# nanoshimarobot/dynamic_direct_lidar_odometry

Measured on AMD Instinct MI355X. Metric: GICP iters/sec + ms/scan, 131k-pt source → 500k-pt submap; pose Δ vs CPU ref, higher is better.
Workload: dtype f32 search / f64 normal equations; 1 GPU; cfg3 S2M GICP: 131,072-pt 64x2048 scan -> 500,000-pt 4-keyframe submap, LM, maxCorr 2.0 m, maxIter 32, transEps 0.01; target_points=500000, parallelism=replicas x1

## Files before the change

### dynamic_direct_lidar_odometry_amd/csrc/moments.hip

```cpp
#include <hip/hip_runtime.h>

#include <cstddef>

#include "gicp_types.hpp"
#include "search.hpp"
#include "nftree.hpp"
#include "cov_math.hpp"
#include "launch.hpp"
#include "launch_util.hpp"
#include "linearize_internal.hpp"
#include "lm_step.hpp"

namespace ddlo {

struct Contrib {
  double M[6];
  double q[3];
  double qq[6];
  double v[3];
  double y;
  double c;
};

template <int S>
__device__ __forceinline__ double moment_val(const Contrib& C) {
  if constexpr (S < 6) {
    return C.M[S];
  } else if constexpr (S < 24) {
    return C.q[(S - 6) / 6] * C.M[(S - 6) % 6];
  } else if constexpr (S < 60) {
    return C.qq[(S - 24) / 6] * C.M[(S - 24) % 6];
  } else if constexpr (S < 72) {
    constexpr int m = (S - 60) / 4, kk = (S - 60) % 4;
    if constexpr (kk == 3)
      return C.v[m];
    else
      return C.v[m] * C.q[kk];
  } else if constexpr (S == 72) {
    return C.y;
  } else if constexpr (S == 73) {
    return C.c;
  } else {
    return 0.0;
  }
}

__device__ __forceinline__ double dpp_f64(double x, int ctrl_sel) {
  const int lo = __double2loint(x), hi = __double2hiint(x);
  int rlo, rhi;
  switch (ctrl_sel) {
    case 0:
      rlo = __builtin_amdgcn_update_dpp(0, lo, 0x140, 0xf, 0xf, false);
      rhi = __builtin_amdgcn_update_dpp(0, hi, 0x140, 0xf, 0xf, false);
      break;
    case 1:
      rlo = __builtin_amdgcn_update_dpp(0, lo, 0x141, 0xf, 0xf, false);
      rhi = __builtin_amdgcn_update_dpp(0, hi, 0x141, 0xf, 0xf, false);
      break;
    case 2:
      rlo = __builtin_amdgcn_update_dpp(0, lo, 0x4e, 0xf, 0xf, false);
      rhi = __builtin_amdgcn_update_dpp(0, hi, 0x4e, 0xf, 0xf, false);
      break;
    default:
      rlo = __builtin_amdgcn_update_dpp(0, lo, 0xb1, 0xf, 0xf, false);
      rhi = __builtin_amdgcn_update_dpp(0, hi, 0xb1, 0xf, 0xf, false);
      break;
  }
  return __hiloint2double(rhi, rlo);
}

template <int L>
__device__ __forceinline__ double xchg(double a, double b) {
  if constexpr (L == 1 || L == 2) {
    const unsigned alo = __double2loint(a), ahi = __double2hiint(a);
    const unsigned blo = __double2loint(b), bhi = __double2hiint(b);
    unsigned x0, x1, y0, y1;
    if constexpr (L == 1) {
      const auto rl = __builtin_amdgcn_permlane32_swap(alo, blo, false, false);
      const auto rh = __builtin_amdgcn_permlane32_swap(ahi, bhi, false, false);
      x0 = rl[0]; y0 = rl[1]; x1 = rh[0]; y1 = rh[1];
    } else {
      const auto rl = __builtin_amdgcn_permlane16_swap(alo, blo, false, false);
      const auto rh = __builtin_amdgcn_permlane16_swap(ahi, bhi, false, false);
      x0 = rl[0]; y0 = rl[1]; x1 = rh[0]; y1 = rh[1];
    }
    return __hiloint2double(x1, x0) + __hiloint2double(y1, y0);
  } else {
    const int bit = 1 << (6 - L);
    const bool hi = (lane_id() & bit) != 0;
    const double keep = hi ? b : a;
    const double send = hi ? a : b;
    return keep + dpp_f64(send, L - 3);
  }
}

template <int L, int S>
__device__ __forceinline__ double treduce(const Contrib& C) {
  if constexpr (L == 0) {
    return moment_val<S>(C);
  } else {
    constexpr int half = kMomentSlots >> L;
    const double a = treduce<L - 1, S>(C);
    const double b = treduce<L - 1, S + half>(C);
    return xchg<L>(a, b);
  }
}

__device__ __forceinline__ double final_pair(double x) { return x + dpp_f64(x, 3); }

__device__ __forceinline__ int moment_base(int lane) {
  return 48 * ((lane >> 5) & 1) + 24 * ((lane >> 4) & 1) + 12 * ((lane >> 3) & 1) + 6 * ((lane >> 2) & 1) +
         3 * ((lane >> 1) & 1);
}

__device__ __forceinline__ void load_sym6(const __attribute__((address_space(1))) double* p, double c[6]) {
  const auto q = (const __attribute__((address_space(1))) d2v*)p;
  const d2v a = q[0];
  const d2v b = q[1];
  const d2v d = q[2];
  c[0] = a.x; c[1] = a.y; c[2] = b.x; c[3] = b.y; c[4] = d.x; c[5] = d.y;
}

constexpr int kMomWaves = 8;

__device__ __forceinline__ void resolve_tied_corr(const AlignJob* __restrict__ job, AlignState* st, const CloudDev& tgt,
                                               bool tied, int i, float kd, int& j, NfWaveStack* S,
                                               bool q_in_regs = false, float qx = 0.f, float qy = 0.f, float qz = 0.f) {
  unsigned long long tm = __ballot(tied);
  const int lane = lane_id();
  const NfTreeDev t = job->tgt_nf;
  if (t.nodes == nullptr) {
    if (lane == __builtin_ctzll(tm)) atomicOr(&st->tie_pending, 1);
    return;
  }
  if (*job->tgt_nf_status) {
    if (lane == __builtin_ctzll(tm)) atomicOr(&st->tie_err, 2);
    return;
  }
  int nres = 0;
  while (tm) {
    const int l = __builtin_ctzll(tm);
    tm &= tm - 1;
    const int il = __builtin_amdgcn_readlane(i, l);
    const float dl = __uint_as_float((unsigned)__builtin_amdgcn_readlane((int)__float_as_uint(kd), l));
    const float4 q = q_in_regs ? make_float4(readlane_f(qx, l), readlane_f(qy, l), readlane_f(qz, l), 0.f)
                               : ldg4(job->qstate, il);
    float rd;
    int rix;
    int err = 0, jn = -1;
    const bool ok = nf_search_wave(t, q.x, q.y, q.z, 1, S, &rd, &rix);
    rd = __uint_as_float((unsigned)__builtin_amdgcn_readfirstlane((int)__float_as_uint(rd)));
    rix = __builtin_amdgcn_readfirstlane(rix);
    if (!ok) err = 1;
    else if (__float_as_uint(rd) != __float_as_uint(dl) || rix < 0 || rix >= t.n) err = 16;
    else if ((jn = tgt.inv_perm[rix]) < 0) err = 32;
    if (lane == l) {
      if (jn >= 0) j = jn;
      else atomicOr(&st->tie_err, err);
    }
    ++nres;
  }
  if (lane == 0) atomicAdd(&st->ties_resolved, nres);
}

#ifndef DDLO_LOOKUP_U
#define DDLO_LOOKUP_U 16
#endif
constexpr int kLookupU = DDLO_LOOKUP_U;

#ifdef DDLO_MOM_PROF
#define MOM_PROF(i) if (LOOKUP) mp_t[i] = __builtin_amdgcn_s_memrealtime()
constexpr int kMomProfIters = 8, kMomProfWaves = 2048;
__device__ unsigned long long g_mom_prof[kMomProfIters * kMomProfWaves * 6];
#else
#define MOM_PROF(i)
#endif
struct TieWords {
  int pending, resolved, err;
};
constexpr int kTieThread = 64 * (kMomWaves - 1);
__device__ __forceinline__ TieWords fetch_tie_words(AlignState* st) {
  TieWords tw{0, 0, 0};
  __hip_atomic_compare_exchange_strong(&st->tie_pending, &tw.pending, 0, __ATOMIC_RELAXED, __ATOMIC_RELAXED,
                                       __HIP_MEMORY_SCOPE_AGENT);
  __hip_atomic_compare_exchange_strong(&st->ties_resolved, &tw.resolved, 0, __ATOMIC_RELAXED, __ATOMIC_RELAXED,
                                       __HIP_MEMORY_SCOPE_AGENT);
  __hip_atomic_compare_exchange_strong(&st->tie_err, &tw.err, 0, __ATOMIC_RELAXED, __ATOMIC_RELAXED,
                                       __HIP_MEMORY_SCOPE_AGENT);
  return tw;
}

__device__ __forceinline__ void publish_state(const AlignJob* __restrict__ job, AlignState* __restrict__ st,
                                              AlignState* __restrict__ publish, const TieWords& tw) {
  static_assert(sizeof(AlignState) % 8 == 0, "AlignState is copied in 8-byte words");
  static_assert(offsetof(AlignState, pub) == sizeof(AlignState) - 8, "the publication word is the last 8 bytes");
  static_assert(offsetof(AlignState, iter) % 8 == 0 && offsetof(AlignState, done) == offsetof(AlignState, iter) + 4,
                "iter and done are one 8-byte word");
  __shared__ int tie_s[3];
  if (threadIdx.x == kTieThread) {
    tie_s[0] = tw.pending;
    tie_s[1] = tw.resolved;
    tie_s[2] = tw.err;
  }
  asm volatile("s_waitcnt vmcnt(0)" ::: "memory");
  __syncthreads();
  const auto src = gpw(reinterpret_cast<unsigned long long*>(st));
  const auto dst = gpw(reinterpret_cast<unsigned long long*>(publish));
  constexpr int kWords = (int)(sizeof(AlignState) / 8);
  static_assert(kWords <= 64 * kMomWaves && kLmThreads == 64 * kMomWaves, "one 8-byte word per thread");
  auto patch = [](unsigned long long v, int w, size_t off, int val) {
    if ((size_t)w != off / 8) return v;
    const int sh = (int)(off & 4) * 8;
    return (v & ~(0xffffffffull << sh)) | ((unsigned long long)(unsigned)val << sh);
  };
  __shared__ unsigned long long iter_s;
  const int w = threadIdx.x;
  if (w < kWords) {
    unsigned long long v = __hip_atomic_load(src + w, __ATOMIC_RELAXED, __HIP_MEMORY_SCOPE_AGENT);
    v = patch(v, w, offsetof(AlignState, tie_pending), tie_s[0]);
    v = patch(v, w, offsetof(AlignState, ties_resolved), tie_s[1]);
    v = patch(v, w, offsetof(AlignState, tie_err), tie_s[2]);
    dst[w] = v;
    if (w == (int)(offsetof(AlignState, iter) / 8)) iter_s = v;
  }
  const unsigned long long tk = job->ticket;
  asm volatile("s_waitcnt vmcnt(0)" ::: "memory");
  __syncthreads();
  if (threadIdx.x == 0) {
    const unsigned long long id = iter_s;
    const unsigned long long w = (tk << 17) | ((unsigned long long)((unsigned)(id >> 32) != 0u) << 16) | (id & 0xffffu);
    __hip_atomic_store(&publish->pub, w, __ATOMIC_RELEASE, __HIP_MEMORY_SCOPE_SYSTEM);
  }
}

template <bool FUSE_LM, bool LOOKUP = false>
__global__ __launch_bounds__(64 * kMomWaves) void k_moments(const AlignJob* __restrict__ job,
                                                            AlignState* __restrict__ st, AlignState* __restrict__ publish) {
#ifdef DDLO_MOM_PROF
  unsigned long long mp_t[6] = {0, 0, 0, 0, 0, 0};
#endif
  MOM_PROF(0);
  const auto sg = gp(st);
  double R[9], t[3];
  for (int e = 0; e < 9; ++e) R[e] = sg->R[e];
  for (int e = 0; e < 3; ++e) t[e] = sg->t[e];
  const int st_rec = sg->rec, st_any_rec = sg->any_rec;
  if (__builtin_amdgcn_readfirstlane(sg->done)) {
    if (FUSE_LM && publish && blockIdx.x == 0) {
      TieWords tw{};
      if (threadIdx.x == kTieThread) tw = fetch_tie_words(st);
      publish_state(job, st, publish, tw);
    }
    return;
  }
  const CloudDev src = job->src;
  const CloudDev tgt = job->tgt;
  const auto src_cov = gp(job->src_cov);
  const auto tgt_cov = gp(job->tgt_cov);
  const auto key = gp((const unsigned long long*)job->key);
  const auto corr = gpw(job->corr);
  const auto sqd = gpw(job->sqd);
  const auto slab = gpw(job->slab);
  const double max_corr2 = job->max_corr2;
  const int rec = st_rec;
  const int first_rec_done = st_any_rec;
  const int tie_detect = job->tie_detect;
  const bool slice_check = tie_detect && job->tie_scan >= 2 && !(job->tie_ab & 4);
  const bool tie3m = tie_detect && job->tie_scan == 3 && !rec;
  __shared__ NfWaveStack tie_stk[kMomWaves];
  const int lane = lane_id();
  const int wib = threadIdx.x >> 6;
#ifdef DDLO_MOM_PROF
  __builtin_amdgcn_s_waitcnt(0);
#endif
  MOM_PROF(1);
  const int wave = blockIdx.x * kMomWaves + wib;
  const int nwaves_total = gridDim.x * kMomWaves;
  const int ngroups = (src.n + 63) >> 6;
  if (blockIdx.x == 0 && threadIdx.x < kTaskRegions) job->task_ctr[threadIdx.x * kCtrStride] = 0u;
  if (blockIdx.x == 0 && job->grid_on && threadIdx.x == 0) {
    unsigned t = 0;
    for (int sg = 0; sg < kFbSegs; ++sg) t += job->fb_count[sg * 32];
    job->fb_count[kFbSegs * 32] += t;
    for (int sg = 0; sg < kFbSegs; ++sg) job->fb_count[sg * 32] = 0u;
  }
  double acc0 = 0.0, acc1 = 0.0, acc2 = 0.0;
  for (int g = wave; g < ngroups; g += nwaves_total) {
    const int i = g * 64 + lane;
    const bool active = i < src.n;
    int j = -1;
    unsigned kj = 0xffffffffu;
    float kd = INFINITY;
    bool tied = false;
    float4 a = make_float4(0.f, 0.f, 0.f, 0.f), b = a;
    double ca[6] = {0, 0, 0, 0, 0, 0}, cb[6] = {0, 0, 0, 0, 0, 0};
    float lqx = 0.f, lqy = 0.f, lqz = 0.f;
    unsigned long long lkey = 0ull;
    unsigned lsec = 0xffffffffu;
    if constexpr (LOOKUP) {
      const CellGridDev G = job->grid;
      a = ldg4(src.pts, active ? i : src.n - 1);
      const float Rf0 = (float)R[0], Rf1 = (float)R[1], Rf2 = (float)R[2], Rf3 = (float)R[3], Rf4 = (float)R[4],
                  Rf5 = (float)R[5], Rf6 = (float)R[6], Rf7 = (float)R[7], Rf8 = (float)R[8];
      const float tf0 = (float)t[0], tf1 = (float)t[1], tf2 = (float)t[2];
      lqx = (Rf0 * a.x + Rf1 * a.y) + (Rf2 * a.z + tf0);
      lqy = (Rf3 * a.x + Rf4 * a.y) + (Rf5 * a.z + tf1);
      lqz = (Rf6 * a.x + Rf7 * a.y) + (Rf8 * a.z + tf2);
      const int g16 = i >> 4;
      const float qa = job->own_axis == 0 ? lqx : job->own_axis == 1 ? lqy : lqz;
      const bool owned = active && (job->own_axis < 0 || (qa >= job->own_lo && qa < job->own_hi)) &&
                         (job->own_mod == 0 || (g16 % job->own_mod) == job->own_rem);
      unsigned off = 0, cnt = 0;
      if (owned) {
        const float tx = (lqx - G.ox) * G.inv_s, ty = (lqy - G.oy) * G.inv_s, tz = (lqz - G.oz) * G.inv_s;
        if (tx >= 0.f && tx < (float)G.nx && ty >= 0.f && ty < (float)G.ny && tz >= 0.f && tz < (float)G.nz) {
          cg_cell_list(G, tx, ty, tz, off, cnt);
        }
      }
      unsigned long long bk = ~0ull;
      float d2 = INFINITY, bx = 0.f, by = 0.f, bz = 0.f;
      const bool track2 = tie_detect;
      constexpr int kU = kLookupU;
      auto consume = [&](const float4 (&pp)[kU], unsigned k) {
#pragma unroll
        for (int u = 0; u < kU; ++u) {
          if (k + u < cnt) {
            const float dd = dist2(lqx, lqy, lqz, pp[u].x, pp[u].y, pp[u].z);
            const unsigned long long kk = dkey(dd, __float_as_int(pp[u].w));
            if (kk < bk) {
              if (track2 && bk != ~0ull) d2 = fminf(d2, __uint_as_float((unsigned)(bk >> 32)));
              bk = kk;
              bx = pp[u].x;
              by = pp[u].y;
              bz = pp[u].z;
            } else if (track2) {
              d2 = fminf(d2, dd);
            }
          }
        }
      };
      auto fetch = [&](float4 (&pp)[kU], unsigned k) {
#pragma unroll
        for (int u = 0; u < kU; ++u) pp[u] = ldg4(G.ent, off + min(k + u, cnt - 1));
      };
      for (unsigned k = 0; k < cnt; k += kU) {
        float4 pp[kU];
        fetch(pp, k);
        consume(pp, k);
      }
      lkey = owned ? umin64(bk, dkey(job->cap2, -1)) : dkey(INFINITY, -1);
      const float lkd = __uint_as_float((unsigned)(lkey >> 32));
      lsec = (owned && (unsigned)lkey != 0xffffffffu && d2 == lkd) ? (unsigned)(lkey >> 32) : 0xffffffffu;
      b = make_float4(bx, by, bz, 0.f);

      MOM_PROF(2);
    }
    if (active) {
      const unsigned long long k = LOOKUP ? lkey : key[i];
      const unsigned sv = !tie_detect ? 0xffffffffu : LOOKUP ? lsec : job->sec[i];
      const unsigned k2lo = (tie3m && !LOOKUP) ? (unsigned)job->key2[i] : 0u;
      kj = (unsigned)k;
      kd = __uint_as_float((unsigned)(k >> 32));
      j = (kj != 0xffffffffu && (double)kd < max_corr2) ? (int)kj : -1;
      if (j >= 0) {
        if constexpr (!LOOKUP) {
          a = ldg4(src.pts, i);
          b = ldg4(tgt.pts, j);
        }

        load_sym6(src_cov + 6 * (size_t)i, ca);
        load_sym6(tgt_cov + 6 * (size_t)j, cb);
      }
      const bool searched = tie_detect && j >= 0 && sv != 0xffffffffu;
      tied = searched && sv <= (unsigned)(k >> 32);
      if (tie3m && searched && !LOOKUP) tied = tied || k2lo != ((unsigned)k ^ 0xffffffffu);
      if (slice_check && searched && !tied) {
        const float qx = ((float)R[0] * a.x + (float)R[1] * a.y) + ((float)R[2] * a.z + (float)t[0]);
        const float qy = ((float)R[3] * a.x + (float)R[4] * a.y) + ((float)R[5] * a.z + (float)t[1]);
        const float qz = ((float)R[6] * a.x + (float)R[7] * a.y) + ((float)R[8] * a.z + (float)t[2]);
        const int b0 = j & ~7;
#pragma unroll
        for (int h = 0; h < 8; ++h) {
          const float4 p = ldg4(tgt.pts, b0 + h);
          tied = tied || (b0 + h != j && dist2(qx, qy, qz, p.x, p.y, p.z) == kd);
        }
      }
    }
    if (tie_detect && __any(tied)) {
      const int j0 = j;
      resolve_tied_corr(job, st, tgt, tied, i, kd, j, &tie_stk[wib], LOOKUP, lqx, lqy, lqz);
      if (tied) kj = (unsigned)j;
      if (j != j0) {
        b = ldg4(tgt.pts, j);
        load_sym6(tgt_cov + 6 * (size_t)j, cb);
      }
    }
    if (active) {
      corr[i] = j;
      sqd[i] = kj != 0xffffffffu ? kd : INFINITY;
      if (rec && !LOOKUP) {
        const float4 qs = ldg4(job->qstate, i);
        if (qs.w >= 0.f) {
          job->ref[i] = make_float4(qs.x, qs.y, qs.z, fminf(__uint_as_float(job->sec[i]), qs.w));
          float4 pp = make_float4(0.f, 0.f, 0.f, __int_as_float(-1));
          if (kj != 0xffffffffu) {
            const float4 p = ldg4(tgt.pts, (int)kj);
            pp = make_float4(p.x, p.y, p.z, __int_as_float((int)kj));
          }
          job->ref_p[i] = pp;
        } else if (!first_rec_done) {
          job->ref[i] = make_float4(0.f, 0.f, 0.f, -1.f);
        }
      }
    }
    Contrib C;
    if (j >= 0) {
      const double A[9] = {ca[0], ca[1], ca[2], ca[1], ca[3], ca[4], ca[2], ca[4], ca[5]};
      double RC[9];
#pragma unroll
      for (int r = 0; r < 3; ++r)
#pragma unroll
        for (int cc = 0; cc < 3; ++cc) RC[3 * r + cc] = R[3 * r] * A[cc] + R[3 * r + 1] * A[3 + cc] + R[3 * r + 2] * A[6 + cc];
      double S[9];
#pragma unroll
      for (int r = 0; r < 3; ++r)
#pragma unroll
        for (int cc = 0; cc < 3; ++cc) S[3 * r + cc] = RC[3 * r] * R[3 * cc] + RC[3 * r + 1] * R[3 * cc + 1] + RC[3 * r + 2] * R[3 * cc + 2];
      const double Cm[9] = {cb[0] + S[0], cb[1] + S[1], cb[2] + S[2], cb[1] + S[3], cb[3] + S[4],
                            cb[4] + S[5], cb[2] + S[6], cb[4] + S[7], cb[5] + S[8]};
      double Mi[9];
      inv3(Cm, Mi);
      C.M[0] = Mi[0]; C.M[1] = 0.5 * (Mi[1] + Mi[3]); C.M[2] = 0.5 * (Mi[2] + Mi[6]);
      C.M[3] = Mi[4]; C.M[4] = 0.5 * (Mi[5] + Mi[7]); C.M[5] = Mi[8];
      const double ax = a.x, ay = a.y, az = a.z;
      C.q[0] = (R[0] * ax + R[1] * ay) + (R[2] * az + t[0]);
      C.q[1] = (R[3] * ax + R[4] * ay) + (R[5] * az + t[1]);
      C.q[2] = (R[6] * ax + R[7] * ay) + (R[8] * az + t[2]);
      const double e0 = (double)b.x - C.q[0], e1 = (double)b.y - C.q[1], e2 = (double)b.z - C.q[2];
      C.v[0] = C.M[0] * e0 + C.M[1] * e1 + C.M[2] * e2;
      C.v[1] = C.M[1] * e0 + C.M[3] * e1 + C.M[4] * e2;
      C.v[2] = C.M[2] * e0 + C.M[4] * e1 + C.M[5] * e2;
      C.y = e0 * C.v[0] + e1 * C.v[1] + e2 * C.v[2];
      C.c = 1.0;
    } else {
      for (int e = 0; e < 6; ++e) C.M[e] = 0.0;
      C.q[0] = C.q[1] = C.q[2] = 0.0;
      C.v[0] = C.v[1] = C.v[2] = 0.0;
      C.y = 0.0;
      C.c = 0.0;
    }
    C.qq[0] = C.q[0] * C.q[0]; C.qq[1] = C.q[0] * C.q[1]; C.qq[2] = C.q[0] * C.q[2];
    C.qq[3] = C.q[1] * C.q[1]; C.qq[4] = C.q[1] * C.q[2]; C.qq[5] = C.q[2] * C.q[2];
    MOM_PROF(3);
    acc0 += final_pair(treduce<5, 0>(C));
    acc1 += final_pair(treduce<5, 1>(C));
    acc2 += final_pair(treduce<5, 2>(C));
  }
  MOM_PROF(4);
  __shared__ double red[kMomWaves][kMomentSlots];
  if ((lane & 1) == 0) {
    const int base = moment_base(lane);
    red[wib][base + 0] = acc0;
    red[wib][base + 1] = acc1;
    red[wib][base + 2] = acc2;
  }
  __syncthreads();
  if (threadIdx.x < kSlabStride) {
    double sum = 0.0;
    if (threadIdx.x < kMoments)
      for (int w = 0; w < kMomWaves; ++w) sum += red[w][threadIdx.x];
    if constexpr (FUSE_LM)
      __hip_atomic_store((__attribute__((address_space(1))) unsigned long long*)(slab + (size_t)blockIdx.x * kSlabStride +
                                                                                 threadIdx.x),
                         (unsigned long long)__double_as_longlong(sum), __ATOMIC_RELAXED, __HIP_MEMORY_SCOPE_AGENT);
    else
      slab[(size_t)blockIdx.x * kSlabStride + threadIdx.x] = sum;
  }
#ifdef DDLO_MOM_PROF
  MOM_PROF(5);
  if (LOOKUP && lane == 0 && wave < kMomProfWaves) {
    unsigned long long* o = g_mom_prof + ((size_t)min(st->iter, kMomProfIters - 1) * kMomProfWaves + wave) * 6;
    for (int e = 0; e < 6; ++e) o[e] = mp_t[e];
  }
#endif
  if constexpr (FUSE_LM) {
    __shared__ int last_s;
    asm volatile("s_waitcnt vmcnt(0)" ::: "memory");
    __syncthreads();
    unsigned* const arrive = job->task_ctr + kTaskRegions * kCtrStride;
    if (threadIdx.x == 0) last_s = atomicAdd(arrive, 1u) == gridDim.x - 1;
    __syncthreads();
    if (!last_s) return;
    if (threadIdx.x == 0) {
      __builtin_amdgcn_fence(__ATOMIC_ACQUIRE, "agent");
      asm volatile("s_waitcnt vmcnt(0)" ::: "memory");
      atomicExch(arrive, 0u);
    }
    __syncthreads();
    TieWords tw{};
    if (publish && threadIdx.x == kTieThread) tw = fetch_tie_words(st);
    lm_step_body<false>(job, st, job->slab, job->nblocks, nullptr);
    if (publish) publish_state(job, st, publish, tw);
  }
}
template __global__ void k_moments<false>(const AlignJob*, AlignState*, AlignState*);
template __global__ void k_moments<true>(const AlignJob*, AlignState*, AlignState*);
template __global__ void k_moments<false, true>(const AlignJob*, AlignState*, AlignState*);
template __global__ void k_moments<true, true>(const AlignJob*, AlignState*, AlignState*);

__global__ __launch_bounds__(kLmThreads) void k_mom_reduce(const AlignJob* __restrict__ job) {
  AlignState* st = job->state;
  if (__builtin_amdgcn_readfirstlane(st->done)) return;
  __shared__ double part[kLmParts][kSlabStride];
  __shared__ double mom[kSlabStride];
  reduce_slab(job->slab, job->nblocks, part, mom);
  __syncthreads();
  if (threadIdx.x < kSlabStride) gpw(job->mom)[threadIdx.x] = mom[threadIdx.x];
}

__global__ __launch_bounds__(kLmThreads) void k_lm_step(const AlignJob* __restrict__ job, AlignState* __restrict__ st,
                                                        const double* __restrict__ slab, int nblocks,
                                                        const double* __restrict__ premom,
                                                        AlignState* __restrict__ publish) {
  TieWords tw{};
  if (publish && threadIdx.x == kTieThread) tw = fetch_tie_words(st);
  if (!__builtin_amdgcn_readfirstlane(st->done)) {
    if (premom) lm_step_body<true>(job, st, slab, nblocks, premom);
    else lm_step_body<false>(job, st, slab, nblocks, nullptr);
  }
  if (publish) publish_state(job, st, publish, tw);
}

void launch_linearize(hipStream_t s, const AlignJob* job, const LinGeom& g, AlignState* publish) {
  static const int fused_lookup = env_knob("DDLO_GRID_FUSED", 1);
  if (g.grid && !g.grid_walk && fused_lookup) {
    if (g.fuse_lm) k_moments<true, true><<<g.mom_blocks, 64 * kMomWaves, 0, s>>>(job, g.state, publish);
    else k_moments<false, true><<<g.mom_blocks, 64 * kMomWaves, 0, s>>>(job, g.state, nullptr);
    return;
  }
  if (g.grid) launch_cell_lookup(s, job, g);
  if (!g.grid || g.grid_walk) launch_nn_walk(s, job, g);
  if (g.fuse_lm) k_moments<true><<<g.mom_blocks, 64 * kMomWaves, 0, s>>>(job, g.state, publish);
  else k_moments<false><<<g.mom_blocks, 64 * kMomWaves, 0, s>>>(job, g.state, nullptr);
}
int moment_blocks(int nsrc) {
  const int groups = (nsrc + 63) / 64;
  return std::max(1, std::min((groups + kMomWaves - 1) / kMomWaves, kMomBlocksMax));
}
int lm_slab_rows_max() { return kMomBlocksMax; }
void launch_lm_step(hipStream_t s, const AlignJob* job, AlignState* st, const double* slab, int nblocks,
                    const double* premom, AlignState* publish) {
  k_lm_step<<<1, kLmThreads, 0, s>>>(job, st, slab, nblocks, premom, publish);
}
void launch_mom_reduce(hipStream_t s, const AlignJob* job) { k_mom_reduce<<<1, kLmThreads, 0, s>>>(job); }

}

#ifdef DDLO_MOM_PROF
extern "C" int ddlo_dev_mom_prof(unsigned long long* out) {
  return (int)hipMemcpyFromSymbol(out, HIP_SYMBOL(ddlo::g_mom_prof), sizeof(ddlo::g_mom_prof));
}
#endif
```

Measured before the change: 31860 GICP iters/s.

## Split heavy-cell candidate scans across lane teams with shuffle merge

Each lane first scans up to the first 32 candidates of its grid cell list. Lanes whose cells hold more candidates are collected per wave by ballot, and each is assigned a power-of-two team of lanes that scan the remaining candidates in strided chunks. Partial bests are merged back through shuffles, keeping the tie-tracking second distance. This aims to cut wave divergence, where a few lanes with long cell lists stall the whole wave, at the cost of extra shuffles and team bookkeeping in the lookup path.

```diff
diff --git a/dynamic_direct_lidar_odometry_amd/csrc/moments.hip b/dynamic_direct_lidar_odometry_amd/csrc/moments.hip
--- a/dynamic_direct_lidar_odometry_amd/csrc/moments.hip
+++ b/dynamic_direct_lidar_odometry_amd/csrc/moments.hip
@@ -167,11 +167,51 @@
 #define DDLO_LOOKUP_U 16
 #endif
 constexpr int kLookupU = DDLO_LOOKUP_U;
+#ifndef DDLO_TAIL_E0
+#define DDLO_TAIL_E0 32
+#endif
+#ifndef DDLO_TAIL_FCAP
+#define DDLO_TAIL_FCAP 64
+#endif
+constexpr unsigned kTailE0 = DDLO_TAIL_E0;
+constexpr int kTailFCap = DDLO_TAIL_FCAP;
+static_assert(kTailE0 > 0 && kTailE0 % kLookupU == 0, "the common rounds end on a round boundary");
+static_assert(kTailFCap >= 1 && kTailFCap <= 64 && (kTailFCap & (kTailFCap - 1)) == 0, "team size: a power of two");
+
+struct LookupBest {
+  unsigned long long bk;
+  float d2, bx, by, bz;
+};
+__device__ __forceinline__ void tail_merge(LookupBest& a, const LookupBest& o, bool track2) {
+  const bool take = o.bk < a.bk;
+  const unsigned long long loser = take ? a.bk : o.bk;
+  if (take) {
+    a.bk = o.bk;
+    a.bx = o.bx;
+    a.by = o.by;
+    a.bz = o.bz;
+  }
+  if (track2) {
+    a.d2 = fminf(a.d2, o.d2);
+    if (loser != ~0ull) a.d2 = fminf(a.d2, __uint_as_float((unsigned)(loser >> 32)));
+  }
+}
+__device__ __forceinline__ LookupBest tail_shfl(const LookupBest& s, int src) {
+  LookupBest r;
+  r.bk = ((unsigned long long)(unsigned)__shfl((int)(unsigned)(s.bk >> 32), src) << 32) |
+         (unsigned)__shfl((int)(unsigned)s.bk, src);
+  r.d2 = __shfl(s.d2, src);
+  r.bx = __shfl(s.bx, src);
+  r.by = __shfl(s.by, src);
+  r.bz = __shfl(s.bz, src);
+  return r;
+}
 
 #ifdef DDLO_MOM_PROF
 #define MOM_PROF(i) if (LOOKUP) mp_t[i] = __builtin_amdgcn_s_memrealtime()
 constexpr int kMomProfIters = 8, kMomProfWaves = 2048;
-__device__ unsigned long long g_mom_prof[kMomProfIters * kMomProfWaves * 6];
+constexpr int kMomProfWords = 7;
+__device__ unsigned long long g_mom_prof[kMomProfIters * kMomProfWaves * kMomProfWords];
 #else
 #define MOM_PROF(i)
 #endif
@@ -237,7 +277,7 @@
 __global__ __launch_bounds__(64 * kMomWaves) void k_moments(const AlignJob* __restrict__ job,
                                                             AlignState* __restrict__ st, AlignState* __restrict__ publish) {
 #ifdef DDLO_MOM_PROF
-  unsigned long long mp_t[6] = {0, 0, 0, 0, 0, 0};
+  unsigned long long mp_t[kMomProfWords] = {0, 0, 0, 0, 0, 0, 0};
 #endif
   MOM_PROF(0);
   const auto sg = gp(st);
@@ -317,37 +357,83 @@
           cg_cell_list(G, tx, ty, tz, off, cnt);
         }
       }
-      unsigned long long bk = ~0ull;
-      float d2 = INFINITY, bx = 0.f, by = 0.f, bz = 0.f;
+      LookupBest own{~0ull, INFINITY, 0.f, 0.f, 0.f};
       const bool track2 = tie_detect;
       constexpr int kU = kLookupU;
-      auto consume = [&](const float4 (&pp)[kU], unsigned k) {
+      auto consume = [&](const float4 (&pp)[kU], unsigned k, unsigned n, float qx, float qy, float qz, LookupBest& r) {
 #pragma unroll
         for (int u = 0; u < kU; ++u) {
-          if (k + u < cnt) {
-            const float dd = dist2(lqx, lqy, lqz, pp[u].x, pp[u].y, pp[u].z);
+          if (k + u < n) {
+            const float dd = dist2(qx, qy, qz, pp[u].x, pp[u].y, pp[u].z);
             const unsigned long long kk = dkey(dd, __float_as_int(pp[u].w));
-            if (kk < bk) {
-              if (track2 && bk != ~0ull) d2 = fminf(d2, __uint_as_float((unsigned)(bk >> 32)));
-              bk = kk;
-              bx = pp[u].x;
-              by = pp[u].y;
-              bz = pp[u].z;
+            if (kk < r.bk) {
+              if (track2 && r.bk != ~0ull) r.d2 = fminf(r.d2, __uint_as_float((unsigned)(r.bk >> 32)));
+              r.bk = kk;
+              r.bx = pp[u].x;
+              r.by = pp[u].y;
+              r.bz = pp[u].z;
             } else if (track2) {
-              d2 = fminf(d2, dd);
+              r.d2 = fminf(r.d2, dd);
             }
           }
         }
       };
-      auto fetch = [&](float4 (&pp)[kU], unsigned k) {
+      auto fetch = [&](float4 (&pp)[kU], unsigned k, unsigned lo, unsigned n) {
 #pragma unroll
-        for (int u = 0; u < kU; ++u) pp[u] = ldg4(G.ent, off + min(k + u, cnt - 1));
+        for (int u = 0; u < kU; ++u) pp[u] = ldg4(G.ent, lo + min(k + u, n - 1));
       };
-      for (unsigned k = 0; k < cnt; k += kU) {
+      const unsigned c0 = min(cnt, kTailE0);
+      for (unsigned k = 0; k < c0; k += kU) {
         float4 pp[kU];
-        fetch(pp, k);
-        consume(pp, k);
+        fetch(pp, k, off, cnt);
+        consume(pp, k, cnt, lqx, lqy, lqz, own);
       }
+      const bool heavy = cnt > kTailE0;
+      const unsigned long long rem = __ballot(heavy);
+      if (rem != 0ull) {
+        const int H = __popcll(rem);
+        int lf = 0;
+        while ((H << (lf + 1)) <= 64 && (2 << lf) <= kTailFCap) ++lf;
+        const int F = 1 << lf;
+        const int rank = __popcll(rem & ((1ull << lane) - 1ull));
+        int owner = lane;
+        if (F > 1) {
+          const int team = lane >> lf;
+          owner = -1;
+          int r = 0;
+          for (unsigned long long mm = rem; mm; mm &= mm - 1, ++r)
+            if (team == r) owner = __builtin_ctzll(mm);
+        }
+        const int osrc = owner < 0 ? lane : owner;
+        const unsigned ooff = (unsigned)__shfl((int)off, osrc);
+        const unsigned ocnt0 = (unsigned)__shfl((int)cnt, osrc);
+        const unsigned ocnt = owner < 0 ? 0u : ocnt0;
+        const float oqx = __shfl(lqx, osrc), oqy = __shfl(lqy, osrc), oqz = __shfl(lqz, osrc);
+        LookupBest mine{~0ull, INFINITY, 0.f, 0.f, 0.f};
+        const unsigned stride = (unsigned)kU << lf;
+        unsigned k = kTailE0 + (unsigned)kU * (unsigned)(lane & (F - 1));
+#ifdef DDLO_MOM_PROF
+        int rounds = 0;
+#define MOM_PROF_ROUND ++rounds
+#else
+#define MOM_PROF_ROUND
+#endif
+        for (; k < ocnt; k += stride) {
+          float4 pp[kU];
+          fetch(pp, k, ooff, ocnt);
+          consume(pp, k, ocnt, oqx, oqy, oqz, mine);
+          MOM_PROF_ROUND;
+        }
+#undef MOM_PROF_ROUND
+        for (int m = 1; m < F; m <<= 1) tail_merge(mine, tail_shfl(mine, lane ^ m), track2);
+        const LookupBest got = tail_shfl(mine, heavy && F > 1 ? rank << lf : lane);
+        if (heavy) tail_merge(own, got, track2);
+#ifdef DDLO_MOM_PROF
+        mp_t[6] = (unsigned long long)H | ((unsigned long long)wave_max((float)rounds) << 8);
+#endif
+      }
+      const unsigned long long bk = own.bk;
+      const float d2 = own.d2, bx = own.bx, by = own.by, bz = own.bz;
       lkey = owned ? umin64(bk, dkey(job->cap2, -1)) : dkey(INFINITY, -1);
       const float lkd = __uint_as_float((unsigned)(lkey >> 32));
       lsec = (owned && (unsigned)lkey != 0xffffffffu && d2 == lkd) ? (unsigned)(lkey >> 32) : 0xffffffffu;
@@ -479,8 +565,8 @@
 #ifdef DDLO_MOM_PROF
   MOM_PROF(5);
   if (LOOKUP && lane == 0 && wave < kMomProfWaves) {
-    unsigned long long* o = g_mom_prof + ((size_t)min(st->iter, kMomProfIters - 1) * kMomProfWaves + wave) * 6;
-    for (int e = 0; e < 6; ++e) o[e] = mp_t[e];
+    unsigned long long* o = g_mom_prof + ((size_t)min(st->iter, kMomProfIters - 1) * kMomProfWaves + wave) * kMomProfWords;
+    for (int e = 0; e < kMomProfWords; ++e) o[e] = mp_t[e];
   }
 #endif
   if constexpr (FUSE_LM) {
```

Result: faster. 33210 GICP iters/s (median of 6 runs) (+4.2%).
